# Jakoebly/marl-sc

Measured on NVIDIA B200. Metric: agent_steps_per_sec_env_step_plus_gae, higher is better.
Workload: dtype uint16 stock+history, uint8 ring / fp32 obs+GAE / fp64 cost sums

## Files before the change

### marl-sc_b200/csrc/env_compact.cu

```cuda
#include "env_compact.cuh"
#include "env_split.cuh"

#ifndef MARLSC_ALLOC_CTAS
#define MARLSC_ALLOC_CTAS 4
#endif
namespace marlsc {
static inline int imin_host(int a, int b) { return a < b ? a : b; }
static inline int imax_host(int a, int b) { return a > b ? a : b; }
namespace {

constexpr unsigned FULL = 0xffffffffu;
constexpr int kSlots = kCompactMaxS / 32;
constexpr int kPlaneBatch = 9;

__device__ __forceinline__ uint32_t sm_addr(const void* p) { return (uint32_t)__cvta_generic_to_shared(p); }
__device__ __forceinline__ uint32_t ld_s_u8(uint32_t a) { uint32_t v; asm volatile("ld.shared.u8 %0, [%1];" : "=r"(v) : "r"(a)); return v; }
__device__ __forceinline__ uint32_t ld_s_u16(uint32_t a) { uint32_t v; asm volatile("ld.shared.u16 %0, [%1];" : "=r"(v) : "r"(a)); return v; }
__device__ __forceinline__ void st_s_u16(uint32_t a, uint32_t v) { asm volatile("st.shared.u16 [%0], %1;" ::"r"(a), "r"(v) : "memory"); }
__device__ __forceinline__ void red_s_add(uint32_t a, uint32_t v) { asm volatile("red.shared.add.u32 [%0], %1;" ::"r"(a), "r"(v) : "memory"); }
__device__ __forceinline__ void red_s_add_f64(uint32_t a, double v) {
  unsigned long long old, seen;
  asm volatile("ld.shared.u64 %0, [%1];" : "=l"(old) : "r"(a) : "memory");
  do {
    seen = old;
    const unsigned long long want = (unsigned long long)__double_as_longlong(__longlong_as_double((long long)seen) + v);
    asm volatile("atom.shared.cas.b64 %0, [%1], %2, %3;" : "=l"(old) : "r"(a), "l"(seen), "l"(want) : "memory");
  } while (old != seen);
}
__device__ __forceinline__ void red_g_add(uint32_t* p, uint32_t v) { asm volatile("red.global.add.u32 [%0], %1;" ::"l"(p), "r"(v) : "memory"); }
__device__ __forceinline__ uint32_t ld_nc_u16(const uint16_t* p) { uint32_t v; asm volatile("ld.global.nc.u16 %0, [%1];" : "=r"(v) : "l"(p)); return v; }
__device__ __forceinline__ uint32_t ld_cg_u16(const uint16_t* p) { uint32_t v; asm volatile("ld.global.cg.u16 %0, [%1];" : "=r"(v) : "l"(p)); return v; }
__device__ __forceinline__ void prefetch_l2_bulk(const void* p, uint32_t bytes) {
  asm volatile("cp.async.bulk.prefetch.L2.global [%0], %1;" ::"l"(p), "r"(bytes) : "memory");
}

__device__ __forceinline__ uint32_t ld_nc_u32(const uint32_t* p) { uint32_t v; asm volatile("ld.global.nc.u32 %0, [%1];" : "=r"(v) : "l"(p)); return v; }
// ... 108 lines not shown
      if (rem != 0u && cand == 0u) {
        red_s_add(a_lostU + 4u * r, rem);
        if (!pen_uniform) red_s_add_f64(a_lostP + 8u * r, (double)rem * sp.pen_rate[sku2 >> 1]);
        rem = 0u;
      }
    }
    if (!__any_sync(FULL, (rem | ls.next()) != 0u)) break;
  }
}

template <bool MS>
__device__ __forceinline__ float nrm(float x, const float* __restrict__ mean, const float* __restrict__ istd, int off) {
  if (MS) return f_mul(f_sub(x, mean[off]), istd[off]);
  return x;
}

#define VALID(k) ((k) < FS || ((k) == FS && tail))

template <int NCH, bool MS, int FS>
__global__ void __launch_bounds__(kCompactWarps * 32, 4)
env_step_compact_kernel(const __grid_constant__ DevSpec sp, const __grid_constant__ marlsc_env_state_t st,
                        const __grid_constant__ marlsc_step_io_t io, int t, int prefetch) {
  extern __shared__ __align__(16) unsigned char smem[];
  __shared__ int s_poff[kCompactMaxL];
  const int W = sp.W, S = sp.S, R = sp.R, L = sp.L, WS = W * S;
  const CompactSmem lay = compact_smem(W, S, R, NCH, sp.pen_uniform);
  if (threadIdx.x < kCompactMaxL) s_poff[threadIdx.x] = (int)((unsigned)(t + 1 + threadIdx.x) % (unsigned)L) * (S >> 2);
  {
    const int n_perm = (R * NCH * 32) >> 1, n_prio = (R * 16) >> 2, n_home = (R + 3) >> 2;
    for (int i = threadIdx.x; i < n_perm + n_prio + n_home; i += blockDim.x) {
      if (i < n_perm) reinterpret_cast<uint32_t*>(smem + lay.t_perm)[i] = reinterpret_cast<const uint32_t*>(sp.perm5)[i];
      else if (i < n_perm + n_prio) reinterpret_cast<uint32_t*>(smem + lay.t_prio)[i - n_perm] = reinterpret_cast<const uint32_t*>(sp.prio16)[i - n_perm];
      else reinterpret_cast<uint32_t*>(smem + lay.t_home)[i - n_perm - n_prio] = reinterpret_cast<const uint32_t*>(sp.home_wh)[i - n_perm - n_prio];
    }
  }
  __syncthreads();
  const int lane = threadIdx.x & 31, wid = threadIdx.x >> 5;
  const int64_t e = (int64_t)blockIdx.x * kCompactWarps + wid;
  if (e >= st.num_envs) return;

  const int64_t round0 = io.line_counts ? e * (int64_t)io.line_stride : (int64_t)io.line_offsets[e];
  const int n_rounds = io.line_counts ? io.line_counts[e] : io.line_offsets[e + 1] - (int)round0;
  if (lane == 0 && n_rounds > 0) prefetch_l2_bulk(io.lines + round0 * 32, (uint32_t)n_rounds * 64u);
  if (prefetch) {
    if (lane == 1) prefetch_l2_bulk(static_cast<const uint8_t*>(st.ring_qty) + e * (int64_t)WS * L, (uint32_t)(WS * L));
    if (lane == 2 && !io.action_qty) prefetch_l2_bulk(io.actions + e * WS, (uint32_t)(WS * 4));
    if (lane == 3) prefetch_l2_bulk(static_cast<const uint16_t*>(st.inventory) + e * WS, (uint32_t)(WS * 2));
    if (lane == 4 && io.action_qty) prefetch_l2_bulk(io.action_qty + e * WS, (uint32_t)WS);
  }

// ... 10 lines not shown
  }

  const bool need_hist = sp.need_hist != 0;
  const int pa = t % L;
  const bool by_row = sp.row_rates_uniform != 0;
  const bool tail = lane < S - 32 * FS;
  uint16_t* const g_inv = pinned(static_cast<uint16_t*>(st.inventory) + e * WS + lane);
  uint8_t* const g_ring = pinned(static_cast<uint8_t*>(st.ring_qty) + e * (int64_t)WS * L + lane);
  uint16_t* const g_hist = need_hist ? pinned(static_cast<uint16_t*>(st.demand_hist) + e * (int64_t)kWindow * WS + lane) : nullptr;
  uint16_t* const hist_now = need_hist ? g_hist + (t % kWindow) * WS : nullptr;
  float* const g_obs = pinned(io.obs + e * (int64_t)W * sp.obs_dim + sp.id_off + lane);
  const float* const mean_l = MS ? sp.obs_mean + lane : nullptr;
  const float* const istd_l = MS ? sp.obs_std + lane : nullptr;
  const int obs_dim = sp.obs_dim, off_pipe = sp.off_pipe, LS = L * S;

  int rowQ = 0, rowPos = 0;
  double rowInb = 0.0;
  {
    const bool mine = 4 * lane < S;
    const int c4 = mine ? lane : 0;
    const float4* __restrict__ act4 = io.action_qty ? nullptr : reinterpret_cast<const float4*>(io.actions + e * WS) + c4;
    const uint32_t* __restrict__ aq4 = io.action_qty ? reinterpret_cast<const uint32_t*>(io.action_qty + e * WS) + c4 : nullptr;
    const uint32_t* __restrict__ lead4 = reinterpret_cast<const uint32_t*>(sp.lead_u8) + c4;
    uint2* inv4 = reinterpret_cast<uint2*>(static_cast<uint16_t*>(st.inventory) + e * WS) + c4;
    uint32_t* row4 = reinterpret_cast<uint32_t*>(static_cast<uint8_t*>(st.ring_qty) + e * (int64_t)WS * L) + c4;
    uint2* hz4 = need_hist ? reinterpret_cast<uint2*>(hist_now - lane) + c4 : nullptr;
    float* __restrict__ out = g_obs + off_pipe;
    float* __restrict__ outc = g_obs - lane + off_pipe + 4 * c4;
    uint32_t a_sinv = sm_addr(s_inv) + 8u * c4;
    const int S4 = S >> 2, LS4 = LS >> 2, pa4 = pa * S4;
    int mx[4];
#pragma unroll
    for (int j = 0; j < 4; ++j) mx[j] = mine ? (int)sp.action_max[4 * lane + j] : 0;
    const int sub = lane & 3, src0 = lane >> 2;
#pragma unroll 1
    for (int w = 0; w < W; ++w) {
      float4 a4 = make_float4(0.f, 0.f, 0.f, 0.f);
      uint32_t aqw = 0u, arr4 = 0u, le4 = 0x01010101u;
      uint2 iv = make_uint2(0u, 0u);
      if (mine) {
        if (aq4) aqw = *aq4; else a4 = *act4;
        iv = *inv4;
        arr4 = row4[pa4];
        le4 = *lead4;
      }
      int q[4], le[4];
      float* dst = out;
      int moff = off_pipe;
#pragma unroll 1
      for (int k0 = 0; k0 < L; k0 += kPlaneBatch) {
        uint32_t x[kPlaneBatch];
#pragma unroll
        for (int kk = 0; kk < kPlaneBatch; ++kk) {
          const bool live = k0 + kk < L - 1;
          x[kk] = (mine && live) ? row4[s_poff[live ? k0 + kk : 0]] : 0u;
        }
        if (k0 == 0) {
          const float af[4] = {a4.x, a4.y, a4.z, a4.w};
          const uint32_t ivv[4] = {iv.x & 0xffffu, iv.x >> 16, iv.y & 0xffffu, iv.y >> 16};
          uint32_t ni[4], newarr = 0u;
          int nQ = 0, nPos = 0;
          double inb = 0.0;
#pragma unroll
          for (int j = 0; j < 4; ++j) {
            le[j] = (int)((le4 >> (8 * j)) & 0xffu);
            q[j] = 0;
            if (mine) q[j] = aq4 ? imin((int)((aqw >> (8 * j)) & 0xffu), mx[j]) : rescale_action<kCapsLean>(sp, af[j], (double)mx[j], 0, 0);
            ni[j] = ivv[j] + ((arr4 >> (8 * j)) & 0xffu);
            if (le[j] == L) newarr |= (uint32_t)q[j] << (8 * j);
            nQ += q[j];
            nPos += q[j] > 0 ? 1 : 0;
            if (!by_row && q[j] > 0) {
              const int i = w * S + 4 * lane + j;
              inb += sp.in_fixed[i] + ((double)q[j] * sp.skw[4 * lane + j]) * sp.in_var[i];
            }
          }
          if (mine) {
            asm volatile("st.shared.v2.u32 [%0], {%1, %2};" ::"r"(a_sinv), "r"(ni[0] | (ni[1] << 16)), "r"(ni[2] | (ni[3] << 16)) : "memory");
            row4[pa4] = newarr;
            uint8_t* rowb = reinterpret_cast<uint8_t*>(row4);
#pragma unroll
            for (int j = 0; j < 4; ++j)
              if (q[j] > 0 && le[j] < L) {
                int p2 = pa + le[j];
                p2 -= p2 >= L ? L : 0;
                rowb[p2 * S + j] = (uint8_t)q[j];
              }
            if (need_hist) *hz4 = make_uint2(0u, 0u);
          }
          if (by_row) {
            nQ = __reduce_add_sync(FULL, nQ);
            nPos = __reduce_add_sync(FULL, nPos);
            if (lane == w) {
              rowQ = nQ;
              rowPos = nPos;
            }
          } else {
#pragma unroll
            for (int o = 16; o > 0; o >>= 1) inb += __shfl_xor_sync(FULL, inb, o);
            if (lane == w) rowInb = inb;
          }
        }
#pragma unroll
        for (int kk = 0; kk < kPlaneBatch; ++kk) {
          if (k0 + kk < L) {
#pragma unroll
            for (int j = 0; j < kSlots; ++j) {
              const uint32_t v = __shfl_sync(FULL, x[kk], 8 * j + src0);
              if (VALID(j)) dst[32 * j] = nrm<MS>((float)((v >> (8 * sub)) & 0xffu), mean_l, istd_l, moff + 32 * j);
            }
            dst += S;
            moff += S;
          }
        }
      }
      if (mine) {
#pragma unroll
        for (int j = 0; j < 4; ++j)
          if (q[j] > 0) {
            const int po = (le[j] - 1) * S + j;
            outc[po] = nrm<MS>((float)q[j], mean_l - lane, istd_l - lane, off_pipe + 4 * lane + po);
          }
      }
      if (aq4) aq4 += S4; else act4 += S4;
      lead4 += S4;
      inv4 += S4;
      row4 += LS4;
      hz4 += S4;
      out += obs_dim;
      outc += obs_dim;
      a_sinv += 2u * S;
    }
  }
  __syncwarp();

  {
    LineStream ls;
    ls.init(io.lines, round0, n_rounds, lane);
    uint32_t avlo, avhi;
    owner_masks(ls.map, sm_addr(s_inv), W, S, avlo, avhi);
    allocation_chains<NCH>(sp, ls, sm_addr(smem + lay.t_perm), sm_addr(smem + lay.t_prio), sm_addr(smem + lay.t_home),
                           sm_addr(s_inv), sm_addr(s_shipq), sm_addr(s_lostU), sm_addr(s_lostP), avlo, avhi,
                           need_hist ? reinterpret_cast<uint32_t*>(hist_now - lane) : nullptr);
  }
  __syncwarp();

  double costA = 0.0;
  {
    const double pen0 = sp.pen_rate[0];
    double rate[2], lump[2];
    int close_w[2];
#pragma unroll
    for (int qq = 0; qq < 2; ++qq) {
// ... 84 lines not shown
#pragma unroll
        for (int o = 16; o > 0; o >>= 1) hold += __shfl_xor_sync(FULL, hold, o);
        if (lane == w) costR = hold + rowInb;
      }
      a_sinv += 2u * S;
      inv += S;
      hnow += S;
#pragma unroll
      for (int back = 1; back < kWindow; ++back) hold_p[back - 1] += S;
      out += obs_dim;
    }
  }

  double rew = lane < W ? -((costR + costA) * sp.scale) : 0.0;
  if (sp.scope == MARLSC_SCOPE_TEAM) {
#pragma unroll
    for (int o = 16; o > 0; o >>= 1) rew += __shfl_xor_sync(FULL, rew, o);
  }
  if (lane < W) io.rewards[e * W + lane] = (float)rew;
  if (io.truncated && lane == 0) io.truncated[e] = (uint8_t)(t + 1 >= sp.episode_length);
}


template <bool MS, bool POLICY, int LT, bool STATS = false>
__global__ void __launch_bounds__(256)
compact_place_kernel(const __grid_constant__ DevSpec sp, const __grid_constant__ marlsc_env_state_t st,
                     const __grid_constant__ marlsc_step_io_t io, double* __restrict__ cost_rows, int t,
                     const __grid_constant__ marlsc_episode_metrics_t m) {
  extern __shared__ __align__(16) unsigned char smem[];
  constexpr int KMAX = LT ? LT : kCompactMaxL;
  const int W = sp.W, S = sp.S, L = LT ? LT : sp.L, WS = W * S;
  const int lane = threadIdx.x & 31;
  const unsigned row = blockIdx.x * 8u + (threadIdx.x >> 5);
  if (row >= (unsigned)st.num_envs * (unsigned)W) return;
  const unsigned eu = row / (unsigned)W;
  const int w = (int)(row - eu * (unsigned)W);
  const int64_t e = eu;
  const bool mine = 4 * lane < S;
  const int c4 = mine ? lane : 0;
  const int S4 = S >> 2, pa = t % L;
  const int LS4 = L * S4;
  int po0 = (pa + 1) * S4;
  po0 = po0 == LS4 ? 0 : po0;
  const bool need_hist = sp.need_hist != 0;
  uint32_t* const row4 = reinterpret_cast<uint32_t*>(static_cast<uint8_t*>(st.ring_qty) + (e * WS + (int64_t)w * S) * L) + c4;
  float4 a4 = make_float4(0.f, 0.f, 0.f, 0.f);
  uint32_t aqw = 0u, arr4 = 0u, le4 = 0x01010101u;
  uint2 iv = make_uint2(0u, 0u);
  uint2* const inv4 = reinterpret_cast<uint2*>(static_cast<uint16_t*>(st.inventory) + e * WS + w * S) + c4;
  uint32_t x[KMAX > 1 ? KMAX - 1 : 1];
  if (mine) {
    if (io.action_qty) aqw = reinterpret_cast<const uint32_t*>(io.action_qty + e * WS + w * S)[c4];
    else if (io.actions) a4 = reinterpret_cast<const float4*>(io.actions + e * WS + w * S)[c4];
    iv = *inv4;
    arr4 = row4[pa * S4];
    le4 = reinterpret_cast<const uint32_t*>(sp.lead_u8 + w * S)[c4];
    int po = po0;
#pragma unroll
    for (int k = 0; k < KMAX - 1; ++k)
      if (k < L - 1) {
        x[k] = row4[po];
        po += S4;
        po = po == LS4 ? 0 : po;
      }
  }
  constexpr bool policy = POLICY;
  float4 lv4 = make_float4(0.f, 0.f, 0.f, 0.f);
  if (policy && mine)
    lv4 = reinterpret_cast<const float4*>(io.base_stock_level + (io.base_stock_per_env ? e * WS : 0) + w * S)[c4];
  const uint32_t img = sm_addr(smem) + (threadIdx.x >> 5) * (uint32_t)(L * S);
  if (mine) {
#pragma unroll
    for (int k = 0; k < KMAX - 1; ++k)
      if (k < L - 1) asm volatile("st.shared.u32 [%0], %1;" ::"r"(img + (uint32_t)(k * S + 4 * lane)), "r"(x[k]) : "memory");
    asm volatile("st.shared.u32 [%0], %1;" ::"r"(img + (uint32_t)((L - 1) * S + 4 * lane)), "r"(0u) : "memory");
  }
  float af[4] = {a4.x, a4.y, a4.z, a4.w};
  const uint32_t ivv[4] = {iv.x & 0xffffu, iv.x >> 16, iv.y & 0xffffu, iv.y >> 16};
  if (policy && mine) {
    const float lv[4] = {lv4.x, lv4.y, lv4.z, lv4.w};
#pragma unroll
    for (int j = 0; j < 4; ++j) {
      uint32_t pend = (arr4 >> (8 * j)) & 0xffu;
#pragma unroll
      for (int k = 0; k < KMAX - 1; ++k)
        if (k < L - 1) pend += (x[k] >> (8 * j)) & 0xffu;
      const double mxd = sp.action_max[4 * lane + j];
      double qd = (double)lv[j] - (double)ivv[j] - (double)pend;
      qd = qd < 0.0 ? 0.0 : (qd > mxd ? mxd : qd);
      af[j] = (float)(2.0 * qd / mxd - 1.0);
    }
  }
  uint32_t ni[4];
  int nQ = 0, nPos = 0;
  double inb = 0.0;
  const bool by_row = sp.row_rates_uniform != 0;
  __syncwarp();
#pragma unroll
  for (int j = 0; j < 4; ++j) {
    const int le = (int)((le4 >> (8 * j)) & 0xffu);
    int q = 0;
    if (mine) {
      const int mxj = (int)sp.action_max[4 * lane + j];
      q = io.action_qty ? imin((int)((aqw >> (8 * j)) & 0xffu), mxj) : rescale_action<kCapsLean>(sp, af[j], (double)mxj, 0, 0);
      if (q > 0) asm volatile("st.shared.u8 [%0], %1;" ::"r"(img + (uint32_t)((le - 1) * S + 4 * lane + j)), "r"(q) : "memory");
    }
    ni[j] = ivv[j] + ((arr4 >> (8 * j)) & 0xffu);
    nQ += q;
    nPos += q > 0 ? 1 : 0;
    if (!by_row && q > 0) {
      const int i = w * S + 4 * lane + j;
      inb += sp.in_fixed[i] + ((double)q * sp.skw[4 * lane + j]) * sp.in_var[i];
    }
  }
  if (mine) {
    *inv4 = make_uint2(ni[0] | (ni[1] << 16), ni[2] | (ni[3] << 16));
    if (need_hist)
      reinterpret_cast<uint2*>(static_cast<uint16_t*>(st.demand_hist) + e * (int64_t)kWindow * WS + (t % kWindow) * WS + w * S)[c4] = make_uint2(0u, 0u);
  }
  if (by_row) {
    nQ = __reduce_add_sync(FULL, nQ);
    nPos = __reduce_add_sync(FULL, nPos);
    if (lane == 0) cost_rows[row] = (double)nPos * sp.in_fixed[w * S] + ((double)nQ * sp.skw[0]) * sp.in_var[w * S];
  } else {
#pragma unroll
    for (int o = 16; o > 0; o >>= 1) inb += __shfl_xor_sync(FULL, inb, o);
    if (lane == 0) cost_rows[row] = inb;
  }
  if (STATS) {
    if (!by_row) nQ = __reduce_add_sync(FULL, nQ);
    if (lane == 0) {
      m.inbound_cost[row] += by_row ? (double)nPos * sp.in_fixed[w * S] + ((double)nQ * sp.skw[0]) * sp.in_var[w * S] : inb;
      m.ordered_units[row] += (double)nQ;
    }
  }
  __syncwarp();
  if (mine) {
    int po = po0;
#pragma unroll
    for (int k = 0; k < KMAX; ++k)
      if (k < L) {
        uint32_t v;
        asm volatile("ld.shared.u32 %0, [%1];" : "=r"(v) : "r"(img + (uint32_t)(k * S + 4 * lane)));
        row4[po] = v;
        po += S4;
        po = po == LS4 ? 0 : po;
      }
  }
  const float* const mean_l = MS ? sp.obs_mean + sp.off_pipe + lane : nullptr;
  const float* const istd_l = MS ? sp.obs_std + sp.off_pipe + lane : nullptr;
  float* const dst = io.obs + (size_t)row * sp.obs_dim + sp.id_off + sp.off_pipe + lane;
  const uint32_t src = img + lane;
  const int n = L * S;
#pragma unroll 4
  for (int i = 0; i < n; i += 32) {
    if (i + lane < n) dst[i] = nrm<MS>((float)ld_s_u8(src + i), mean_l, istd_l, i);
  }
}

template <int NCH, int FS, bool STATS = false>
__global__ void __launch_bounds__(kCompactWarps * 32, MARLSC_ALLOC_CTAS)
compact_alloc_kernel(const __grid_constant__ DevSpec sp, const __grid_constant__ marlsc_env_state_t st,
                     const __grid_constant__ marlsc_step_io_t io, const __grid_constant__ CompactSmem lay,
                     double* __restrict__ cost_alloc, int t, const __grid_constant__ marlsc_episode_metrics_t m) {
  extern __shared__ __align__(16) unsigned char smem[];
  const int W = sp.W, S = sp.S, R = sp.R, WS = W * S;
  {
    const int n_perm = (R * NCH * 32) >> 1, n_prio = (R * 16) >> 2, n_home = (R + 3) >> 2;
    for (int i = threadIdx.x; i < n_perm + n_prio + n_home; i += blockDim.x) {
      if (i < n_perm) reinterpret_cast<uint32_t*>(smem + lay.t_perm)[i] = reinterpret_cast<const uint32_t*>(sp.perm5)[i];
      else if (i < n_perm + n_prio) reinterpret_cast<uint32_t*>(smem + lay.t_prio)[i - n_perm] = reinterpret_cast<const uint32_t*>(sp.prio16)[i - n_perm];
      else reinterpret_cast<uint32_t*>(smem + lay.t_home)[i - n_perm - n_prio] = reinterpret_cast<const uint32_t*>(sp.home_wh)[i - n_perm - n_prio];
    }
  }
  __syncthreads();
  const int lane = threadIdx.x & 31, wid = threadIdx.x >> 5;
  const int64_t e = (int64_t)blockIdx.x * kCompactWarps + wid;
  if (e >= st.num_envs) return;
  const bool tail = lane < S - 32 * FS;
  const int64_t round0 = io.line_counts ? e * (int64_t)io.line_stride : (int64_t)io.line_offsets[e];
// ... 389 lines not shown
    uint16_t* h = static_cast<uint16_t*>(st.demand_hist) + e * (long long)kWindow * WS + i;
    for (int b = 0; b < kWindow; ++b) h[b * WS] = 0;
  }
  const bool ms = sp.norm == MARLSC_NORM_MEANSTD;
  float* obs_w = obs + (e * W + w) * (long long)sp.obs_dim;
  float* out = obs_w + sp.id_off;
  put(sp, ms, out, (unsigned)(sp.off_inv + s), (float)v);
  for (int k = 0; k < L; ++k) put(sp, ms, out, (unsigned)(sp.off_pipe + k * S + s), 0.f);
  if (sp.off_dh >= 0) put(sp, ms, out, (unsigned)(sp.off_dh + s), 0.f);
  if (sp.off_rm >= 0) put(sp, ms, out, (unsigned)(sp.off_rm + s), 0.f);
  if (s == 0) {
    if (sp.feat & MARLSC_F_INVENTORY_AGG) {
      int tot = 0;
      for (int ss = 0; ss < S; ++ss) tot += init[(per_env ? e * WS : 0) + w * S + ss];
      put(sp, ms, out, (unsigned)(sp.off_inv + S), (float)tot);
    }
    for (int j = 0; j < sp.id_off; ++j) obs_w[j] = j == w ? 1.0f : 0.0f;
  }
}

template <typename IDX>
__global__ void __launch_bounds__(256)
base_stock_compact_kernel(const __grid_constant__ DevSpec sp, const __grid_constant__ marlsc_env_state_t st,
                          const float* __restrict__ level, int level_per_env, float* __restrict__ actions) {
  const IDX WS = (IDX)(sp.W * sp.S);
  const IDX idx = (IDX)blockIdx.x * (IDX)blockDim.x + (IDX)threadIdx.x;
  if (idx >= (IDX)st.num_envs * WS) return;
  const IDX e = idx / WS;
  const int i = (int)(idx - e * WS), w = i / sp.S, s = i - w * sp.S;
  const int L = sp.L;
  const uint8_t* ring = static_cast<const uint8_t*>(st.ring_qty) + ((long long)e * (long long)WS + (long long)w * sp.S) * L + s;
  int pending = 0;
  for (int d0 = 0; d0 < L; d0 += 4) {
    int v[4];
#pragma unroll
    for (int k = 0; k < 4; ++k) v[k] = d0 + k < L ? (int)ring[(d0 + k) * sp.S] : 0;
    pending += (v[0] + v[1]) + (v[2] + v[3]);
  }
  const double mx = sp.action_max[s];
  double q = (double)(level_per_env ? level[idx] : level[i]) - (double)static_cast<const uint16_t*>(st.inventory)[idx] - (double)pending;
  q = q < 0.0 ? 0.0 : (q > mx ? mx : q);
  actions[idx] = (float)(2.0 * q / mx - 1.0);
}

__global__ void __launch_bounds__(128)
lines_from_orders_kernel(const __grid_constant__ DevSpec sp, long long E, const __grid_constant__ marlsc_step_io_t io,
                         int stride, uint16_t* __restrict__ lines, int32_t* __restrict__ counts, int32_t* __restrict__ overflow) {
  __shared__ uint16_t s_cnt[4][128];
  __shared__ uint16_t s_base[4][128];
  __shared__ uint8_t s_dst[4][128];
  __shared__ uint8_t s_map[4][128];
  __shared__ uint16_t s_dcnt[4][128];
  const int wid = threadIdx.x >> 5;
  const long long e = (long long)blockIdx.x * 4 + wid;
  if (e >= E) return;
  const int lane = threadIdx.x & 31, S = sp.S;
  const long long o_begin = io.order_counts ? e * (long long)io.order_stride : (long long)io.order_offsets[e];
  const int n_orders = io.order_counts ? io.order_counts[e] : io.order_offsets[e + 1] - (int)o_begin;
  const uint8_t* qty = static_cast<const uint8_t*>(io.order_qty) + o_begin * S + lane;
// ... 74 lines not shown
          if (at[k] < stride) env_lines[(long long)(at[k] >> 1) * 64 + 2 * dl[k] + (at[k] & 1)] = line_entry((int)v[jj][k], r, ds[k]);
          else over = true;
          ++at[k];
        }
    }
  }
  const int longest = __reduce_max_sync(FULL, total);
  int rounds = 0;
  if (longest > 0) {
    const int mine = imin(total + 2, stride);
    rounds = (imin(longest + 2, stride) + 1) & ~1;
    uint16_t* const out = env_lines + 2 * lane;
    out[0] = (uint16_t)(map & 0xffffu);
    out[1] = (uint16_t)(map >> 16);
    for (int p = mine; p < rounds; ++p) out[(long long)(p >> 1) * 64 + (p & 1)] = 0;
  }
  if (lane == 0) counts[e] = rounds;
  if (over) atomicExch(overflow, 1);
}

template <int NCH, bool MS, int FS>
int launch_step_nch(const LaunchArgs& a, const marlsc_step_io_t& io, int t, cudaStream_t s) {
  const CompactSmem lay = compact_smem(a.ds.W, a.ds.S, a.ds.R, NCH, a.ds.pen_uniform);
  const size_t smem = (size_t)lay.t_bytes + (size_t)kCompactWarps * lay.warp_bytes;
  if ((int)smem > a.max_smem_optin)
    return set_error(MARLSC_EUNSUPPORTED, "compact step: shared-memory scratch of " + std::to_string(smem) + " bytes per CTA does not fit");
  static int configured_for[kMaxDevices] = {0};
  int dev = 0;
  MARLSC_CUDA(cudaGetDevice(&dev));
  if (dev >= kMaxDevices || configured_for[dev] < (int)smem) {
    MARLSC_CUDA(cudaFuncSetAttribute((const void*)env_step_compact_kernel<NCH, MS, FS>, cudaFuncAttributePreferredSharedMemoryCarveout,
                                     (int)cudaSharedmemCarveoutMaxShared));
    MARLSC_CUDA(cudaFuncSetAttribute((const void*)env_step_compact_kernel<NCH, MS, FS>, cudaFuncAttributeMaxDynamicSharedMemorySize, (int)smem));
    if (dev < kMaxDevices) configured_for[dev] = (int)smem;
  }
  const unsigned grid = (unsigned)((a.st.num_envs + kCompactWarps - 1) / kCompactWarps);
  const auto al16 = [](const void* p) { return (reinterpret_cast<uintptr_t>(p) & 15u) == 0; };
  const int prefetch = a.ds.compact_prefetch && al16(a.st.ring_qty) && al16(a.st.inventory) && al16(io.actions) && al16(io.action_qty);
  env_step_compact_kernel<NCH, MS, FS><<<grid, kCompactWarps * 32, smem, s>>>(a.ds, a.st, io, t, prefetch);
  g_launches.fetch_add(1, std::memory_order_relaxed);
  MARLSC_CUDA(cudaGetLastError());
  return MARLSC_OK;
}

template <int NCH, bool MS, int FS>
int launch_split_nch(const LaunchArgs& a, const marlsc_step_io_t& io, const SplitWork& wk, int t, cudaStream_t s) {
  const CompactSmem lay = compact_smem(a.ds.W, a.ds.S, a.ds.R, NCH, a.ds.pen_uniform);
// ... 6 lines not shown
  if (dev >= kMaxDevices || configured_for[dev] < (int)smem) {
    MARLSC_CUDA(cudaFuncSetAttribute((const void*)compact_alloc_kernel<NCH, FS>, cudaFuncAttributePreferredSharedMemoryCarveout,
                                     (int)cudaSharedmemCarveoutMaxShared));
    MARLSC_CUDA(cudaFuncSetAttribute((const void*)compact_alloc_kernel<NCH, FS>, cudaFuncAttributeMaxDynamicSharedMemorySize, (int)smem));
    if (dev < kMaxDevices) configured_for[dev] = (int)smem;
  }
  const bool stats = wk.metrics != nullptr;
  const marlsc_episode_metrics_t m = stats ? *wk.metrics : marlsc_episode_metrics_t{};
  if (stats) {
    static int stats_configured_for[kMaxDevices] = {0};
    if (dev >= kMaxDevices || stats_configured_for[dev] < (int)smem) {
      MARLSC_CUDA(cudaFuncSetAttribute((const void*)compact_alloc_kernel<NCH, FS, true>, cudaFuncAttributePreferredSharedMemoryCarveout,
                                       (int)cudaSharedmemCarveoutMaxShared));
      MARLSC_CUDA(cudaFuncSetAttribute((const void*)compact_alloc_kernel<NCH, FS, true>, cudaFuncAttributeMaxDynamicSharedMemorySize, (int)smem));
      if (dev < kMaxDevices) stats_configured_for[dev] = (int)smem;
    }
  }
  const int64_t rows = a.st.num_envs * a.ds.W;
  const unsigned grid_rows = (unsigned)((rows + 7) / 8);
  const unsigned grid_envs = (unsigned)((a.st.num_envs + kCompactWarps - 1) / kCompactWarps);
  if (wk.marks) MARLSC_CUDA(cudaEventRecord(wk.marks[0], s));
  {
    const bool policy = !io.actions && !io.action_qty;
    const size_t img = (size_t)8 * a.ds.L * a.ds.S;
#define MARLSC_PLACE_L(LT)                                                                                          \
  case LT:                                                                                                          \
    if (policy) compact_place_kernel<MS, true, LT><<<grid_rows, 256, img, s>>>(a.ds, a.st, io, wk.cost_rows, t, m);  \
    else compact_place_kernel<MS, false, LT><<<grid_rows, 256, img, s>>>(a.ds, a.st, io, wk.cost_rows, t, m);        \
    break;
    if (stats) {
      if (policy) compact_place_kernel<MS, true, 0, true><<<grid_rows, 256, img, s>>>(a.ds, a.st, io, wk.cost_rows, t, m);
      else compact_place_kernel<MS, false, 0, true><<<grid_rows, 256, img, s>>>(a.ds, a.st, io, wk.cost_rows, t, m);
    } else switch (a.ds.L) {
      MARLSC_PLACE_L(1) MARLSC_PLACE_L(2) MARLSC_PLACE_L(3) MARLSC_PLACE_L(4) MARLSC_PLACE_L(5) MARLSC_PLACE_L(6)
      MARLSC_PLACE_L(7) MARLSC_PLACE_L(8) MARLSC_PLACE_L(9) MARLSC_PLACE_L(10) MARLSC_PLACE_L(11) MARLSC_PLACE_L(12)
      MARLSC_PLACE_L(13) MARLSC_PLACE_L(14) MARLSC_PLACE_L(15) MARLSC_PLACE_L(16)
      default:
        if (policy) compact_place_kernel<MS, true, 0><<<grid_rows, 256, img, s>>>(a.ds, a.st, io, wk.cost_rows, t, m);
        else compact_place_kernel<MS, false, 0><<<grid_rows, 256, img, s>>>(a.ds, a.st, io, wk.cost_rows, t, m);
    }
#undef MARLSC_PLACE_L
  }
  MARLSC_CUDA(cudaGetLastError());
  if (wk.marks) MARLSC_CUDA(cudaEventRecord(wk.marks[1], s));
  if (stats) compact_alloc_kernel<NCH, FS, true><<<grid_envs, kCompactWarps * 32, smem, s>>>(a.ds, a.st, io, lay, wk.cost_alloc, t, m);
  else compact_alloc_kernel<NCH, FS><<<grid_envs, kCompactWarps * 32, smem, s>>>(a.ds, a.st, io, lay, wk.cost_alloc, t, m);
  MARLSC_CUDA(cudaGetLastError());
// ... 67 lines not shown
}

int launch_split_compact(const LaunchArgs& a, const marlsc_step_io_t& io, const SplitWork& wk, int t, cudaStream_t s) {
  const bool ms = a.ds.norm == MARLSC_NORM_MEANSTD;
  switch (a.ds.perm5_chunks) {
    case 1: return ms ? launch_split_fs<1, true>(a, io, wk, t, s) : launch_split_fs<1, false>(a, io, wk, t, s);
    case 2: return ms ? launch_split_fs<2, true>(a, io, wk, t, s) : launch_split_fs<2, false>(a, io, wk, t, s);
    case 3: return ms ? launch_split_fs<3, true>(a, io, wk, t, s) : launch_split_fs<3, false>(a, io, wk, t, s);
    case 4: return ms ? launch_split_fs<4, true>(a, io, wk, t, s) : launch_split_fs<4, false>(a, io, wk, t, s);
    default: return set_error(MARLSC_EUNSUPPORTED, "compact step needs W <= 16");
  }
}

int launch_reset_compact(const LaunchArgs& a, const int32_t* init, int per_env, float* obs, cudaStream_t s) {
  const long long n = a.st.num_envs * (long long)a.ds.W * a.ds.S;
  env_reset_compact_kernel<<<(unsigned)((n + 255) / 256), 256, 0, s>>>(a.ds, a.st, init, per_env, obs);
  g_launches.fetch_add(1, std::memory_order_relaxed);
  MARLSC_CUDA(cudaGetLastError());
  return MARLSC_OK;
}

int launch_base_stock_compact(const DevSpec& ds, const marlsc_env_state_t& st, const float* level, int level_per_env, int t,
                              float* actions, cudaStream_t s) {
  (void)t;
  const long long n = st.num_envs * (long long)ds.W * ds.S;
  const unsigned grid = (unsigned)((n + 255) / 256);
  if (n < (1LL << 32)) base_stock_compact_kernel<unsigned><<<grid, 256, 0, s>>>(ds, st, level, level_per_env, actions);
  else base_stock_compact_kernel<long long><<<grid, 256, 0, s>>>(ds, st, level, level_per_env, actions);
  g_launches.fetch_add(1, std::memory_order_relaxed);
  MARLSC_CUDA(cudaGetLastError());
  return MARLSC_OK;
}

int launch_lines_from_orders(const DevSpec& ds, int64_t num_envs, const marlsc_step_io_t& io, int32_t line_stride, uint16_t* lines,
                             int32_t* line_counts, int32_t* overflow, cudaStream_t s) {
  lines_from_orders_kernel<<<(unsigned)((num_envs + 3) / 4), 128, 0, s>>>(ds, num_envs, io, line_stride, lines, line_counts, overflow);
  g_launches.fetch_add(1, std::memory_order_relaxed);
  MARLSC_CUDA(cudaGetLastError());
  return MARLSC_OK;
}

}
```

### marl-sc_b200/envs/batched_env.py

```python
from __future__ import annotations

import ctypes as C
from typing import Any, Dict, List, Optional, Sequence, Tuple, Union

import numpy as np
import torch

from .. import _capi
from ..config.schema import (EnvironmentConfig, InitialInventoryCustom, InitialInventoryUniform,
                             InitialInventoryZero)
from ..demand import LineBatch, OrderBatch, pack_lines, pack_orders
from ..seeds import ENVIRONMENT_SEEDS, SeedManager
from ..spec import EnvSpec, build_env_spec


def _ptr(t: Optional[torch.Tensor]) -> Optional[int]:
    return None if t is None else t.data_ptr()


METRICS_PER_ROW = ("holding_cost", "penalty_cost", "outbound_cost", "inbound_cost", "ordered_units", "shipped_units",
                   "episode_return")
METRICS_PER_ENV = ("demand_units", "lost_units")
COST_METRICS = ("holding_cost", "penalty_cost", "outbound_cost", "inbound_cost")

# ... 10 lines not shown
    @property
    def qty_bytes(self) -> int:
        return self.qty.element_size()

    @staticmethod
    def from_host(batch: OrderBatch, device) -> "DeviceOrders":
        region = batch.region if batch.region.size else np.zeros(1, np.int16)
        qty = torch.from_numpy(batch.qty.view(np.uint8)).to(device)
        if batch.qty_bytes == 2:
            qty = qty.view(torch.int16)
        return DeviceOrders(torch.from_numpy(batch.offsets).to(device), torch.from_numpy(region).to(device),
                            qty, batch.n_orders)


class DeviceLines:

    def __init__(self, offsets: torch.Tensor, lines: torch.Tensor, n_lines: int, n_rounds: int):
        self.offsets, self.lines, self.n_lines, self.n_rounds = offsets, lines, int(n_lines), int(n_rounds)

    @staticmethod
    def from_host(batch: LineBatch, device) -> "DeviceLines":
        return DeviceLines(torch.from_numpy(batch.offsets).to(device), torch.from_numpy(batch.lines.view(np.int16)).to(device),
                           batch.n_lines, batch.n_rounds)


class BatchedInventoryEnv:
    metadata = {"render_modes": ["human"], "name": "multi_env"}

    def __init__(self, env_config: EnvironmentConfig, num_envs: int, device: Union[str, torch.device, None] = None,
                 seed: Optional[int] = None, env_meta: Optional[Dict[str, Any]] = None,
                 region_map: Optional[Sequence[int]] = None, env_seeds: Optional[Sequence[int]] = None,
                 host_samplers: bool = True, diagnostics: bool = False, team_size: int = 0,
                 generic_kernel: bool = False, fused_kernel: bool = False, device_demand: bool = False, demand_seed: int = 0,
                 max_orders_per_env: Optional[int] = None, layout: Optional[str] = None, episode_metrics: bool = False):
        if num_envs < 1:
            raise ValueError("num_envs must be positive")
        if episode_metrics and fused_kernel and layout == "compact":
            raise ValueError("episode_metrics needs the compact layout's split step: the fused kernel does not accumulate them")
        if not torch.cuda.is_available():
            raise RuntimeError("BatchedInventoryEnv needs a CUDA device: this path has no CPU implementation")
        meta = env_meta or {}
        self.env_config = env_config
        self.num_envs = int(num_envs)
        self.device = torch.device(device if device is not None else f"cuda:{torch.cuda.current_device()}")
        if self.device.type != "cuda":
            raise ValueError("device must be a CUDA device")
# ... 292 lines not shown
        _capi.check(_capi.lib().marlsc_env_set_timing(self._h, int(on)))

    def last_step_timing(self) -> list:
        buf = (C.c_float * 8)()
        n = _capi.lib().marlsc_env_last_timing(self._h, buf, 8)
        if n < 0:
            _capi.check(n)
        return [float(buf[i]) for i in range(n)]

    def _compute_local_obs_dim(self) -> int:
        return self.obs_dim

    def agent_observations(self, obs: Optional[torch.Tensor] = None) -> torch.Tensor:
        o = self.obs if obs is None else obs
        E, W, D = o.shape
        return torch.cat([o, o.reshape(E, 1, W * D).expand(E, W, W * D)], dim=2)

    def global_state(self, obs: Optional[torch.Tensor] = None) -> torch.Tensor:
        o = self.obs if obs is None else obs
        return o.reshape(o.shape[0], -1)

    def pending_matrix(self) -> torch.Tensor:
        if self.layout == "compact":
            return self.ring_qty.sum(dim=2, dtype=torch.int32).to(torch.float32)
        t = self.timestep
        D = self.ring_depth
        tau = torch.tensor([t - 1 - ((t - 1 - d) % D) for d in range(D)], device=self.device).view(1, D, 1, 1)
        if self.stochastic_lead:
            lead = self.ring_lead.to(torch.int64)
        else:
            lead = torch.from_numpy(self.expected_lead_times).to(self.device).view(1, 1, *self.expected_lead_times.shape).to(torch.int64)
        live = (tau >= 0) & (self.ring_qty > 0) & (tau + lead >= t)
        return (self.ring_qty * live).sum(dim=1).to(torch.float32)

    def _initial_inventory(self) -> Tuple[torch.Tensor, int]:
        W, S = self.n_warehouses, self.n_skus
        ic = self.env_config.initial_inventory
        if isinstance(ic, InitialInventoryUniform):
            lo, hi = ic.params["min"], ic.params["max"]
            if self._host_samplers:
                vals = np.stack([sm.get_rng("inventory").integers(lo, hi + 1, size=(W, S)) for sm in self.seed_managers])
                return torch.from_numpy(vals.astype(np.int32)).to(self.device), 1
            g = torch.Generator(device=self.device)
            g.manual_seed((int(self._seed or 0) * 1000003 + self._episode) & 0x7fffffffffffffff)
            return torch.randint(lo, hi + 1, (self.num_envs, W, S), dtype=torch.int32, device=self.device, generator=g), 1
        if isinstance(ic, InitialInventoryCustom):
            v = ic.params["values"]
# ... 245 lines not shown
```

Baseline: 375.7 million.

## Store ring orders by placement time and rebuild pipeline from shared image

Changes the compact ring buffer so each slot holds the order placed at that timestep instead of scattering quantities to their arrival slot. Arrivals are read at offset lead from a per-warp shared-memory image, and the pipeline observation is rebuilt per SKU from that image. This removes the scattered byte writes and the shuffle-based plane transposition. In exchange it adds shared memory per warp, reads that depend on lead time, and matching changes to the base-stock and pending-matrix logic.

```diff
diff --git a/marl-sc_b200/csrc/env_compact.cu b/marl-sc_b200/csrc/env_compact.cu
--- a/marl-sc_b200/csrc/env_compact.cu
+++ b/marl-sc_b200/csrc/env_compact.cu
@@ -12,6 +12,7 @@
 constexpr unsigned FULL = 0xffffffffu;
 constexpr int kSlots = kCompactMaxS / 32;
 constexpr int kPlaneBatch = 9;
+__host__ __device__ inline int fused_image_bytes(int L, int S) { return ((L + 1) * S + 15) & ~15; }
 
 __device__ __forceinline__ uint32_t sm_addr(const void* p) { return (uint32_t)__cvta_generic_to_shared(p); }
 __device__ __forceinline__ uint32_t ld_s_u8(uint32_t a) { uint32_t v; asm volatile("ld.shared.u8 %0, [%1];" : "=r"(v) : "r"(a)); return v; }
@@ -166,10 +167,8 @@
 env_step_compact_kernel(const __grid_constant__ DevSpec sp, const __grid_constant__ marlsc_env_state_t st,
                         const __grid_constant__ marlsc_step_io_t io, int t, int prefetch) {
   extern __shared__ __align__(16) unsigned char smem[];
-  __shared__ int s_poff[kCompactMaxL];
   const int W = sp.W, S = sp.S, R = sp.R, L = sp.L, WS = W * S;
   const CompactSmem lay = compact_smem(W, S, R, NCH, sp.pen_uniform);
-  if (threadIdx.x < kCompactMaxL) s_poff[threadIdx.x] = (int)((unsigned)(t + 1 + threadIdx.x) % (unsigned)L) * (S >> 2);
   {
     const int n_perm = (R * NCH * 32) >> 1, n_prio = (R * 16) >> 2, n_home = (R + 3) >> 2;
     for (int i = threadIdx.x; i < n_perm + n_prio + n_home; i += blockDim.x) {
@@ -226,113 +225,106 @@
     const float4* __restrict__ act4 = io.action_qty ? nullptr : reinterpret_cast<const float4*>(io.actions + e * WS) + c4;
     const uint32_t* __restrict__ aq4 = io.action_qty ? reinterpret_cast<const uint32_t*>(io.action_qty + e * WS) + c4 : nullptr;
     const uint32_t* __restrict__ lead4 = reinterpret_cast<const uint32_t*>(sp.lead_u8) + c4;
+    const uint8_t* __restrict__ lead_l = sp.lead_u8 + lane;
     uint2* inv4 = reinterpret_cast<uint2*>(static_cast<uint16_t*>(st.inventory) + e * WS) + c4;
     uint32_t* row4 = reinterpret_cast<uint32_t*>(static_cast<uint8_t*>(st.ring_qty) + e * (int64_t)WS * L) + c4;
     uint2* hz4 = need_hist ? reinterpret_cast<uint2*>(hist_now - lane) + c4 : nullptr;
     float* __restrict__ out = g_obs + off_pipe;
-    float* __restrict__ outc = g_obs - lane + off_pipe + 4 * c4;
     uint32_t a_sinv = sm_addr(s_inv) + 8u * c4;
+    const uint32_t img = sm_addr(smem + lay.t_bytes) + (uint32_t)(kCompactWarps * lay.warp_bytes + wid * fused_image_bytes(L, S));
     const int S4 = S >> 2, LS4 = LS >> 2, pa4 = pa * S4;
     int mx[4];
 #pragma unroll
     for (int j = 0; j < 4; ++j) mx[j] = mine ? (int)sp.action_max[4 * lane + j] : 0;
-    const int sub = lane & 3, src0 = lane >> 2;
 #pragma unroll 1
     for (int w = 0; w < W; ++w) {
       float4 a4 = make_float4(0.f, 0.f, 0.f, 0.f);
-      uint32_t aqw = 0u, arr4 = 0u, le4 = 0x01010101u;
+      uint32_t aqw = 0u, le4 = 0x01010101u;
       uint2 iv = make_uint2(0u, 0u);
       if (mine) {
         if (aq4) aqw = *aq4; else a4 = *act4;
         iv = *inv4;
-        arr4 = row4[pa4];
         le4 = *lead4;
       }
-      int q[4], le[4];
-      float* dst = out;
-      int moff = off_pipe;
+      int lo[kSlots];
+#pragma unroll
+      for (int j = 0; j < kSlots; ++j) lo[j] = VALID(j) ? (int)lead_l[32 * j] : 0;
+      int po = pa4;
 #pragma unroll 1
       for (int k0 = 0; k0 < L; k0 += kPlaneBatch) {
         uint32_t x[kPlaneBatch];
 #pragma unroll
         for (int kk = 0; kk < kPlaneBatch; ++kk) {
-          const bool live = k0 + kk < L - 1;
-          x[kk] = (mine && live) ? row4[s_poff[live ? k0 + kk : 0]] : 0u;
-        }
-        if (k0 == 0) {
-          const float af[4] = {a4.x, a4.y, a4.z, a4.w};
-          const uint32_t ivv[4] = {iv.x & 0xffffu, iv.x >> 16, iv.y & 0xffffu, iv.y >> 16};
-          uint32_t ni[4], newarr = 0u;
-          int nQ = 0, nPos = 0;
-          double inb = 0.0;
-#pragma unroll
-          for (int j = 0; j < 4; ++j) {
-            le[j] = (int)((le4 >> (8 * j)) & 0xffu);
-            q[j] = 0;
-            if (mine) q[j] = aq4 ? imin((int)((aqw >> (8 * j)) & 0xffu), mx[j]) : rescale_action<kCapsLean>(sp, af[j], (double)mx[j], 0, 0);
-            ni[j] = ivv[j] + ((arr4 >> (8 * j)) & 0xffu);
-            if (le[j] == L) newarr |= (uint32_t)q[j] << (8 * j);
-            nQ += q[j];
-            nPos += q[j] > 0 ? 1 : 0;
-            if (!by_row && q[j] > 0) {
-              const int i = w * S + 4 * lane + j;
-              inb += sp.in_fixed[i] + ((double)q[j] * sp.skw[4 * lane + j]) * sp.in_var[i];
-            }
+          x[kk] = (mine && k0 + kk < L) ? row4[po] : 0u;
+          po += S4;
+          po = po >= LS4 ? po - LS4 : po;
+        }
+        if (mine) {
+#pragma unroll
+          for (int kk = 0; kk < kPlaneBatch; ++kk)
+            if (k0 + kk < L) asm volatile("st.shared.u32 [%0], %1;" ::"r"(img + (uint32_t)((k0 + kk) * S + 4 * lane)), "r"(x[kk]) : "memory");
+        }
+      }
+      {
+        const float af[4] = {a4.x, a4.y, a4.z, a4.w};
+        const uint32_t ivv[4] = {iv.x & 0xffffu, iv.x >> 16, iv.y & 0xffffu, iv.y >> 16};
+        uint32_t ni[4], nw = 0u;
+        int nQ = 0, nPos = 0;
+        double inb = 0.0;
+#pragma unroll
+        for (int j = 0; j < 4; ++j) {
+          const int le = (int)((le4 >> (8 * j)) & 0xffu);
+          int q = 0;
+          uint32_t arr = 0u;
+          if (mine) {
+            q = aq4 ? imin((int)((aqw >> (8 * j)) & 0xffu), mx[j]) : rescale_action<kCapsLean>(sp, af[j], (double)mx[j], 0, 0);
+            arr = ld_s_u8(img + (uint32_t)((L - le) * S + 4 * lane + j));
           }
-          if (mine) {
-            asm volatile("st.shared.v2.u32 [%0], {%1, %2};" ::"r"(a_sinv), "r"(ni[0] | (ni[1] << 16)), "r"(ni[2] | (ni[3] << 16)) : "memory");
-            row4[pa4] = newarr;
-            uint8_t* rowb = reinterpret_cast<uint8_t*>(row4);
-#pragma unroll
-            for (int j = 0; j < 4; ++j)
-              if (q[j] > 0 && le[j] < L) {
-                int p2 = pa + le[j];
-                p2 -= p2 >= L ? L : 0;
-                rowb[p2 * S + j] = (uint8_t)q[j];
-              }
-            if (need_hist) *hz4 = make_uint2(0u, 0u);
+          nw |= (uint32_t)q << (8 * j);
+          ni[j] = ivv[j] + arr;
+          nQ += q;
+          nPos += q > 0 ? 1 : 0;
+          if (!by_row && q > 0) {
+            const int i = w * S + 4 * lane + j;
+            inb += sp.in_fixed[i] + ((double)q * sp.skw[4 * lane + j]) * sp.in_var[i];
           }
-          if (by_row) {
-            nQ = __reduce_add_sync(FULL, nQ);
-            nPos = __reduce_add_sync(FULL, nPos);
-            if (lane == w) {
-              rowQ = nQ;
-              rowPos = nPos;
-            }
-          } else {
-#pragma unroll
-            for (int o = 16; o > 0; o >>= 1) inb += __shfl_xor_sync(FULL, inb, o);
-            if (lane == w) rowInb = inb;
+        }
+        if (mine) {
+          asm volatile("st.shared.v2.u32 [%0], {%1, %2};" ::"r"(a_sinv), "r"(ni[0] | (ni[1] << 16)), "r"(ni[2] | (ni[3] << 16)) : "memory");
+          asm volatile("st.shared.u32 [%0], %1;" ::"r"(img + (uint32_t)(L * S + 4 * lane)), "r"(nw) : "memory");
+          row4[pa4] = nw;
+          if (need_hist) *hz4 = make_uint2(0u, 0u);
+        }
+        if (by_row) {
+          nQ = __reduce_add_sync(FULL, nQ);
+          nPos = __reduce_add_sync(FULL, nPos);
+          if (lane == w) {
+            rowQ = nQ;
+            rowPos = nPos;
           }
-        }
-#pragma unroll
-        for (int kk = 0; kk < kPlaneBatch; ++kk) {
-          if (k0 + kk < L) {
-#pragma unroll
-            for (int j = 0; j < kSlots; ++j) {
-              const uint32_t v = __shfl_sync(FULL, x[kk], 8 * j + src0);
-              if (VALID(j)) dst[32 * j] = nrm<MS>((float)((v >> (8 * sub)) & 0xffu), mean_l, istd_l, moff + 32 * j);
-            }
-            dst += S;
-            moff += S;
-          }
-        }
-      }
-      if (mine) {
-#pragma unroll
-        for (int j = 0; j < 4; ++j)
-          if (q[j] > 0) {
-            const int po = (le[j] - 1) * S + j;
-            outc[po] = nrm<MS>((float)q[j], mean_l - lane, istd_l - lane, off_pipe + 4 * lane + po);
-          }
-      }
+        } else {
+#pragma unroll
+          for (int o = 16; o > 0; o >>= 1) inb += __shfl_xor_sync(FULL, inb, o);
+          if (lane == w) rowInb = inb;
+        }
+      }
+      __syncwarp();
+#pragma unroll 1
+      for (int k = 0; k < L; ++k) {
+#pragma unroll
+        for (int j = 0; j < kSlots; ++j) {
+          const uint32_t v = k < lo[j] ? ld_s_u8(img + (uint32_t)((L + 1 - lo[j] + k) * S + lane + 32 * j)) : 0u;
+          if (VALID(j)) out[k * S + 32 * j] = nrm<MS>((float)v, mean_l, istd_l, off_pipe + k * S + 32 * j);
+        }
+      }
+      __syncwarp();
       if (aq4) aq4 += S4; else act4 += S4;
       lead4 += S4;
+      lead_l += S;
       inv4 += S4;
       row4 += LS4;
       hz4 += S4;
       out += obs_dim;
-      outc += obs_dim;
       a_sinv += 2u * S;
     }
   }
@@ -463,6 +455,7 @@
 }
 
 
+constexpr int kPlaceRow = kCompactMaxS;
 template <bool MS, bool POLICY, int LT, bool STATS = false>
 __global__ void __launch_bounds__(256)
 compact_place_kernel(const __grid_constant__ DevSpec sp, const __grid_constant__ marlsc_env_state_t st,
@@ -479,74 +472,76 @@
   const int64_t e = eu;
   const bool mine = 4 * lane < S;
   const int c4 = mine ? lane : 0;
-  const int S4 = S >> 2, pa = t % L;
-  const int LS4 = L * S4;
-  int po0 = (pa + 1) * S4;
-  po0 = po0 == LS4 ? 0 : po0;
+  const int S4 = S >> 2, pa = t % L, LS4 = L * S4;
   const bool need_hist = sp.need_hist != 0;
   uint32_t* const row4 = reinterpret_cast<uint32_t*>(static_cast<uint8_t*>(st.ring_qty) + (e * WS + (int64_t)w * S) * L) + c4;
   float4 a4 = make_float4(0.f, 0.f, 0.f, 0.f);
-  uint32_t aqw = 0u, arr4 = 0u, le4 = 0x01010101u;
+  uint32_t aqw = 0u, le4 = 0x01010101u;
   uint2 iv = make_uint2(0u, 0u);
   uint2* const inv4 = reinterpret_cast<uint2*>(static_cast<uint16_t*>(st.inventory) + e * WS + w * S) + c4;
-  uint32_t x[KMAX > 1 ? KMAX - 1 : 1];
+  uint32_t x[KMAX];
   if (mine) {
     if (io.action_qty) aqw = reinterpret_cast<const uint32_t*>(io.action_qty + e * WS + w * S)[c4];
     else if (io.actions) a4 = reinterpret_cast<const float4*>(io.actions + e * WS + w * S)[c4];
     iv = *inv4;
-    arr4 = row4[pa * S4];
     le4 = reinterpret_cast<const uint32_t*>(sp.lead_u8 + w * S)[c4];
-    int po = po0;
-#pragma unroll
-    for (int k = 0; k < KMAX - 1; ++k)
-      if (k < L - 1) {
+    int po = pa * S4;
+#pragma unroll
+    for (int k = 0; k < KMAX; ++k)
+      if (k < L) {
         x[k] = row4[po];
         po += S4;
         po = po == LS4 ? 0 : po;
       }
   }
+  int lo[kSlots];
+#pragma unroll
+  for (int j = 0; j < kSlots; ++j) lo[j] = lane + 32 * j < S ? (int)sp.lead_u8[w * S + lane + 32 * j] : 1;
   constexpr bool policy = POLICY;
   float4 lv4 = make_float4(0.f, 0.f, 0.f, 0.f);
   if (policy && mine)
     lv4 = reinterpret_cast<const float4*>(io.base_stock_level + (io.base_stock_per_env ? e * WS : 0) + w * S)[c4];
-  const uint32_t img = sm_addr(smem) + (threadIdx.x >> 5) * (uint32_t)(L * S);
+  const uint32_t img = sm_addr(smem) + (threadIdx.x >> 5) * (uint32_t)(2 * L * kPlaceRow);
   if (mine) {
 #pragma unroll
-    for (int k = 0; k < KMAX - 1; ++k)
-      if (k < L - 1) asm volatile("st.shared.u32 [%0], %1;" ::"r"(img + (uint32_t)(k * S + 4 * lane)), "r"(x[k]) : "memory");
-    asm volatile("st.shared.u32 [%0], %1;" ::"r"(img + (uint32_t)((L - 1) * S + 4 * lane)), "r"(0u) : "memory");
-  }
+    for (int k = 0; k < KMAX; ++k)
+      if (k < L) asm volatile("st.shared.u32 [%0], %1;" ::"r"(img + (uint32_t)(k * kPlaceRow + 4 * lane)), "r"(x[k]) : "memory");
+  }
+  for (int o = 16 * lane; o < (L - 1) * kPlaceRow; o += 512)
+    asm volatile("st.shared.v4.u32 [%0], {%1, %1, %1, %1};" ::"r"(img + (uint32_t)((L + 1) * kPlaceRow + o)), "r"(0u) : "memory");
   float af[4] = {a4.x, a4.y, a4.z, a4.w};
   const uint32_t ivv[4] = {iv.x & 0xffffu, iv.x >> 16, iv.y & 0xffffu, iv.y >> 16};
   if (policy && mine) {
     const float lv[4] = {lv4.x, lv4.y, lv4.z, lv4.w};
 #pragma unroll
     for (int j = 0; j < 4; ++j) {
-      uint32_t pend = (arr4 >> (8 * j)) & 0xffu;
-#pragma unroll
-      for (int k = 0; k < KMAX - 1; ++k)
-        if (k < L - 1) pend += (x[k] >> (8 * j)) & 0xffu;
+      const int le = (int)((le4 >> (8 * j)) & 0xffu);
+      uint32_t pend = 0u;
+#pragma unroll
+      for (int k = 0; k < KMAX; ++k)
+        if (k < L && k >= L - le) pend += (x[k] >> (8 * j)) & 0xffu;
       const double mxd = sp.action_max[4 * lane + j];
       double qd = (double)lv[j] - (double)ivv[j] - (double)pend;
       qd = qd < 0.0 ? 0.0 : (qd > mxd ? mxd : qd);
       af[j] = (float)(2.0 * qd / mxd - 1.0);
     }
   }
-  uint32_t ni[4];
+  uint32_t ni[4], nw = 0u;
   int nQ = 0, nPos = 0;
   double inb = 0.0;
   const bool by_row = sp.row_rates_uniform != 0;
-  __syncwarp();
 #pragma unroll
   for (int j = 0; j < 4; ++j) {
     const int le = (int)((le4 >> (8 * j)) & 0xffu);
     int q = 0;
+    uint32_t arr = 0u;
     if (mine) {
       const int mxj = (int)sp.action_max[4 * lane + j];
       q = io.action_qty ? imin((int)((aqw >> (8 * j)) & 0xffu), mxj) : rescale_action<kCapsLean>(sp, af[j], (double)mxj, 0, 0);
-      if (q > 0) asm volatile("st.shared.u8 [%0], %1;" ::"r"(img + (uint32_t)((le - 1) * S + 4 * lane + j)), "r"(q) : "memory");
-    }
-    ni[j] = ivv[j] + ((arr4 >> (8 * j)) & 0xffu);
+      arr = ld_s_u8(img + (uint32_t)((L - le) * kPlaceRow + 4 * lane + j));
+    }
+    nw |= (uint32_t)q << (8 * j);
+    ni[j] = ivv[j] + arr;
     nQ += q;
     nPos += q > 0 ? 1 : 0;
     if (!by_row && q > 0) {
@@ -555,6 +550,8 @@
     }
   }
   if (mine) {
+    asm volatile("st.shared.u32 [%0], %1;" ::"r"(img + (uint32_t)(L * kPlaceRow + 4 * lane)), "r"(nw) : "memory");
+    row4[pa * S4] = nw;
     *inv4 = make_uint2(ni[0] | (ni[1] << 16), ni[2] | (ni[3] << 16));
     if (need_hist)
       reinterpret_cast<uint2*>(static_cast<uint16_t*>(st.demand_hist) + e * (int64_t)kWindow * WS + (t % kWindow) * WS + w * S)[c4] = make_uint2(0u, 0u);
@@ -576,27 +573,19 @@
     }
   }
   __syncwarp();
-  if (mine) {
-    int po = po0;
-#pragma unroll
-    for (int k = 0; k < KMAX; ++k)
-      if (k < L) {
-        uint32_t v;
-        asm volatile("ld.shared.u32 %0, [%1];" : "=r"(v) : "r"(img + (uint32_t)(k * S + 4 * lane)));
-        row4[po] = v;
-        po += S4;
-        po = po == LS4 ? 0 : po;
-      }
-  }
   const float* const mean_l = MS ? sp.obs_mean + sp.off_pipe + lane : nullptr;
   const float* const istd_l = MS ? sp.obs_std + sp.off_pipe + lane : nullptr;
   float* const dst = io.obs + (size_t)row * sp.obs_dim + sp.id_off + sp.off_pipe + lane;
-  const uint32_t src = img + lane;
-  const int n = L * S;
-#pragma unroll 4
-  for (int i = 0; i < n; i += 32) {
-    if (i + lane < n) dst[i] = nrm<MS>((float)ld_s_u8(src + i), mean_l, istd_l, i);
-  }
+  uint32_t src[kSlots];
+#pragma unroll
+  for (int j = 0; j < kSlots; ++j) src[j] = img + (uint32_t)((L + 1 - lo[j]) * kPlaceRow + lane + 32 * j);
+#pragma unroll
+  for (int k = 0; k < KMAX; ++k)
+    if (k < L) {
+#pragma unroll
+      for (int j = 0; j < kSlots; ++j)
+        if (lane + 32 * j < S) dst[k * S + 32 * j] = nrm<MS>((float)ld_s_u8(src[j] + (uint32_t)(k * kPlaceRow)), mean_l, istd_l, k * S + 32 * j);
+    }
 }
 
 template <int NCH, int FS, bool STATS = false>
@@ -1032,19 +1021,22 @@
 template <typename IDX>
 __global__ void __launch_bounds__(256)
 base_stock_compact_kernel(const __grid_constant__ DevSpec sp, const __grid_constant__ marlsc_env_state_t st,
-                          const float* __restrict__ level, int level_per_env, float* __restrict__ actions) {
+                          const float* __restrict__ level, int level_per_env, int t, float* __restrict__ actions) {
   const IDX WS = (IDX)(sp.W * sp.S);
   const IDX idx = (IDX)blockIdx.x * (IDX)blockDim.x + (IDX)threadIdx.x;
   if (idx >= (IDX)st.num_envs * WS) return;
   const IDX e = idx / WS;
   const int i = (int)(idx - e * WS), w = i / sp.S, s = i - w * sp.S;
-  const int L = sp.L;
+  const int L = sp.L, le = sp.lead_u8[i];
   const uint8_t* ring = static_cast<const uint8_t*>(st.ring_qty) + ((long long)e * (long long)WS + (long long)w * sp.S) * L + s;
-  int pending = 0;
-  for (int d0 = 0; d0 < L; d0 += 4) {
+  int pending = 0, p = pmod(t - le, L);
+  for (int a0 = 0; a0 < le; a0 += 4) {
     int v[4];
 #pragma unroll
-    for (int k = 0; k < 4; ++k) v[k] = d0 + k < L ? (int)ring[(d0 + k) * sp.S] : 0;
+    for (int k = 0; k < 4; ++k) {
+      v[k] = a0 + k < le ? (int)ring[p * sp.S] : 0;
+      p = p + 1 == L ? 0 : p + 1;
+    }
     pending += (v[0] + v[1]) + (v[2] + v[3]);
   }
   const double mx = sp.action_max[s];
@@ -1165,7 +1157,7 @@
 template <int NCH, bool MS, int FS>
 int launch_step_nch(const LaunchArgs& a, const marlsc_step_io_t& io, int t, cudaStream_t s) {
   const CompactSmem lay = compact_smem(a.ds.W, a.ds.S, a.ds.R, NCH, a.ds.pen_uniform);
-  const size_t smem = (size_t)lay.t_bytes + (size_t)kCompactWarps * lay.warp_bytes;
+  const size_t smem = (size_t)lay.t_bytes + (size_t)kCompactWarps * (lay.warp_bytes + fused_image_bytes(a.ds.L, a.ds.S));
   if ((int)smem > a.max_smem_optin)
     return set_error(MARLSC_EUNSUPPORTED, "compact step: shared-memory scratch of " + std::to_string(smem) + " bytes per CTA does not fit");
   static int configured_for[kMaxDevices] = {0};
@@ -1218,7 +1210,7 @@
   if (wk.marks) MARLSC_CUDA(cudaEventRecord(wk.marks[0], s));
   {
     const bool policy = !io.actions && !io.action_qty;
-    const size_t img = (size_t)8 * a.ds.L * a.ds.S;
+    const size_t img = (size_t)8 * 2 * a.ds.L * kPlaceRow;
 #define MARLSC_PLACE_L(LT)                                                                                          \
   case LT:                                                                                                          \
     if (policy) compact_place_kernel<MS, true, LT><<<grid_rows, 256, img, s>>>(a.ds, a.st, io, wk.cost_rows, t, m);  \
@@ -1332,11 +1324,10 @@
 
 int launch_base_stock_compact(const DevSpec& ds, const marlsc_env_state_t& st, const float* level, int level_per_env, int t,
                               float* actions, cudaStream_t s) {
-  (void)t;
   const long long n = st.num_envs * (long long)ds.W * ds.S;
   const unsigned grid = (unsigned)((n + 255) / 256);
-  if (n < (1LL << 32)) base_stock_compact_kernel<unsigned><<<grid, 256, 0, s>>>(ds, st, level, level_per_env, actions);
-  else base_stock_compact_kernel<long long><<<grid, 256, 0, s>>>(ds, st, level, level_per_env, actions);
+  if (n < (1LL << 32)) base_stock_compact_kernel<unsigned><<<grid, 256, 0, s>>>(ds, st, level, level_per_env, t, actions);
+  else base_stock_compact_kernel<long long><<<grid, 256, 0, s>>>(ds, st, level, level_per_env, t, actions);
   g_launches.fetch_add(1, std::memory_order_relaxed);
   MARLSC_CUDA(cudaGetLastError());
   return MARLSC_OK;
diff --git a/marl-sc_b200/envs/batched_env.py b/marl-sc_b200/envs/batched_env.py
--- a/marl-sc_b200/envs/batched_env.py
+++ b/marl-sc_b200/envs/batched_env.py
@@ -56,6 +56,13 @@
     def from_host(batch: LineBatch, device) -> "DeviceLines":
         return DeviceLines(torch.from_numpy(batch.offsets).to(device), torch.from_numpy(batch.lines.view(np.int16)).to(device),
                            batch.n_lines, batch.n_rounds)
+
+
+def compact_in_transit(ring_qty: torch.Tensor, lead: torch.Tensor, timestep: int) -> torch.Tensor:
+    Lm = ring_qty.shape[2]
+    age = (timestep - 1 - torch.arange(Lm, device=ring_qty.device)) % Lm
+    live = age.view(1, Lm, 1) < lead.to(ring_qty.device).unsqueeze(1)
+    return (ring_qty.to(torch.int32) * live).sum(dim=2, dtype=torch.int32)
 
 
 class BatchedInventoryEnv:
@@ -394,7 +401,8 @@
 
     def pending_matrix(self) -> torch.Tensor:
         if self.layout == "compact":
-            return self.ring_qty.sum(dim=2, dtype=torch.int32).to(torch.float32)
+            lead = torch.from_numpy(np.ascontiguousarray(self.expected_lead_times, dtype=np.int64)).to(self.device)
+            return compact_in_transit(self.ring_qty, lead, self.timestep).to(torch.float32)
         t = self.timestep
         D = self.ring_depth
         tau = torch.tensor([t - 1 - ((t - 1 - d) % D) for d in range(D)], device=self.device).view(1, D, 1, 1)
```

Measured after the change: 364.3 million (median of 6 runs). 0.969x the previous value.
